# orishu/kraken

Hardware: AMD Instinct MI355X
Metric: metainfo+digest GB/s (device-resident & end-to-end) at 1/2/4/8 MI355X (higher is better)
Workload: dtype u8

## Files before the change

### kraken_amd/csrc/sha256_multi.hip

```cpp
#include <stdlib.h>

#include <atomic>
#include <mutex>

#include "../../include/kraken_hip_internal.h"
#include "kernels.hpp"
#include "knobs.hpp"
#include "device_util.hpp"

namespace krk {

#define KRK_K256                                                                                 \
    0x428a2f98u, 0x71374491u, 0xb5c0fbcfu, 0xe9b5dba5u, 0x3956c25bu, 0x59f111f1u, 0x923f82a4u,     \
        0xab1c5ed5u, 0xd807aa98u, 0x12835b01u, 0x243185beu, 0x550c7dc3u, 0x72be5d74u, 0x80deb1feu, \
        0x9bdc06a7u, 0xc19bf174u, 0xe49b69c1u, 0xefbe4786u, 0x0fc19dc6u, 0x240ca1ccu, 0x2de92c6fu, \
        0x4a7484aau, 0x5cb0a9dcu, 0x76f988dau, 0x983e5152u, 0xa831c66du, 0xb00327c8u, 0xbf597fc7u, \
        0xc6e00bf3u, 0xd5a79147u, 0x06ca6351u, 0x14292967u, 0x27b70a85u, 0x2e1b2138u, 0x4d2c6dfcu, \
        0x53380d13u, 0x650a7354u, 0x766a0abbu, 0x81c2c92eu, 0x92722c85u, 0xa2bfe8a1u, 0xa81a664bu, \
        0xc24b8b70u, 0xc76c51a3u, 0xd192e819u, 0xd6990624u, 0xf40e3585u, 0x106aa070u, 0x19a4c116u, \
        0x1e376c08u, 0x2748774cu, 0x34b0bcb5u, 0x391c0cb3u, 0x4ed8aa4au, 0x5b9cca4fu, 0x682e6ff3u, \
        0x748f82eeu, 0x78a5636fu, 0x84c87814u, 0x8cc70208u, 0x90befffau, 0xa4506cebu, 0xbef9a3f7u, \
        0xc67178f2u

__device__ __forceinline__ uint32_t rotr(uint32_t x, uint32_t n) {
    return __builtin_amdgcn_alignbit(x, x, n);
}
__device__ __forceinline__ uint32_t bswap(uint32_t x) { return __builtin_bswap32(x); }

#ifdef KRK_DIAG
__device__ __forceinline__ void compress(uint32_t h[8], uint32_t w[16]) {
    constexpr uint32_t K[64] = {KRK_K256};
    uint32_t a = h[0], b = h[1], c = h[2], d = h[3], e = h[4], f = h[5], g = h[6], hh = h[7];
#pragma unroll
    for (int i = 0; i < 64; ++i) {
        uint32_t wi;
        if (i < 16) {
            wi = w[i];
        } else {
            const uint32_t w15 = w[(i - 15) & 15], w2 = w[(i - 2) & 15];
            const uint32_t s0 = xor3(rotr(w15, 7), rotr(w15, 18), w15 >> 3);
            const uint32_t s1 = xor3(rotr(w2, 17), rotr(w2, 19), w2 >> 10);
            wi = w[i & 15] + s0 + w[(i - 7) & 15] + s1;
            w[i & 15] = wi;
        }
        const uint32_t S1 = xor3(rotr(e, 6), rotr(e, 11), rotr(e, 25));
        const uint32_t ch = (e & f) ^ (~e & g);
        const uint32_t t1 = hh + S1 + ch + K[i] + wi;
        const uint32_t S0 = xor3(rotr(a, 2), rotr(a, 13), rotr(a, 22));
        const uint32_t mj = __builtin_amdgcn_bitop3_b32(a, b, c, 0xE8);
        const uint32_t t2 = S0 + mj;
        hh = g; g = f; f = e; e = d + t1; d = c; c = b; b = a; a = t1 + t2;
    }
    h[0] += a; h[1] += b; h[2] += c; h[3] += d; h[4] += e; h[5] += f; h[6] += g; h[7] += hh;
}

__device__ __forceinline__ void load_block(uint64_t p, bool al16, uint32_t w[16], uint64_t lo = 0,
                                           uint64_t hi = ~0ull) {
    if (al16) {
        gptr<u32x4> q = as_global<u32x4>(p);
#pragma unroll
        for (int k = 0; k < 4; ++k) {
            const u32x4 v = KRK_GUARD(p + 16 * k, 16, lo, hi, 2) ? q[k] : u32x4{0, 0, 0, 0};
            w[4 * k + 0] = bswap(v.x); w[4 * k + 1] = bswap(v.y);
            w[4 * k + 2] = bswap(v.z); w[4 * k + 3] = bswap(v.w);
        }
    } else {
        load_bytes64(p, 64, w, lo, hi);
#pragma unroll
        for (int k = 0; k < 16; ++k) w[k] = bswap(w[k]);
    }
}

__global__ void __launch_bounds__(64)
sha256_multi_kernel(const ShaJob* __restrict__ jobs, uint32_t n_jobs, uint8_t* __restrict__ out_digest,
                    uint32_t* __restrict__ out_state) {
    const uint32_t j = blockIdx.x * 64 + threadIdx.x;
    if (j >= n_jobs) return;
    const ShaJob job = jobs[j];
    const uint64_t p = job.ptr;
    const bool al16 = (job.ptr & 15) == 0;
    const uint64_t lo = p & ~uint64_t(3), hi = (p + job.len + 3) & ~uint64_t(3);
    uint32_t h[8];
    if (job.flags & kShaFromState) {
#pragma unroll
        for (int k = 0; k < 8; ++k) h[k] = out_state[8 * (uint64_t)job.out + k];
    } else {
// ... 181 lines not shown
#define KRK_SHA_ROUND(A, B, C, D, E, F, G, HK, KWN, NE, NA, NH)                  \
    "v_alignbit_b32 %[r6], %[" #E "], %[" #E "], 6\n\t"                        \
    "v_alignbit_b32 %[r11], %[" #E "], %[" #E "], 11\n\t"                      \
    "v_alignbit_b32 %[r25], %[" #E "], %[" #E "], 25\n\t"                      \
    "v_bitop3_b32 %[ch], %[" #E "], %[" #F "], %[" #G "] bitop3:0xca\n\t"     \
    "v_bitop3_b32 %[r6], %[r6], %[r11], %[r25] bitop3:0x96\n\t"                \
    "v_alignbit_b32 %[q2], %[" #A "], %[" #A "], 2\n\t"                        \
    "v_add3_u32 %[t1], %[" #HK "], %[r6], %[ch]\n\t"                           \
    "v_alignbit_b32 %[q13], %[" #A "], %[" #A "], 13\n\t"                      \
    "v_add_u32_e32 %[" #NE "], %[" #D "], %[t1]\n\t"                           \
    "v_alignbit_b32 %[q22], %[" #A "], %[" #A "], 22\n\t"                      \
    "v_bitop3_b32 %[mj], %[" #A "], %[" #B "], %[" #C "] bitop3:0xe8\n\t"     \
    "v_bitop3_b32 %[q2], %[q2], %[q13], %[q22] bitop3:0x96\n\t"                \
    "v_add_u32_e32 %[" #NH "], %[" #G "], %[" #KWN "]\n\t"                     \
    "v_add3_u32 %[" #NA "], %[t1], %[q2], %[mj]\n\t"

__device__ __forceinline__ void sha_quad(uint32_t& a, uint32_t& b, uint32_t& c, uint32_t& d, uint32_t& e,
                                         uint32_t& f, uint32_t& g, uint32_t& hk, uint32_t k1, uint32_t k2,
                                         uint32_t k3, uint32_t k4, uint32_t& h_last) {
    uint32_t r6, r11, r25, ch, q2, t1, q13, q22, mj;
    uint32_t e1, e2, e3, e4, a1, a2, a3, a4, h1, h2, h3, h4;
    asm volatile(KRK_SHA_ROUND(a, b, c, d, e, f, g, hk, k1, e1, a1, h1)
                 KRK_SHA_ROUND(a1, a, b, c, e1, e, f, h1, k2, e2, a2, h2)
                 KRK_SHA_ROUND(a2, a1, a, b, e2, e1, e, h2, k3, e3, a3, h3)
                 KRK_SHA_ROUND(a3, a2, a1, a, e3, e2, e1, h3, k4, e4, a4, h4)
                 : [r6] "=&v"(r6), [r11] "=&v"(r11), [r25] "=&v"(r25), [ch] "=&v"(ch), [q2] "=&v"(q2),
                   [t1] "=&v"(t1), [q13] "=&v"(q13), [q22] "=&v"(q22), [mj] "=&v"(mj), [e1] "=&v"(e1),
                   [e2] "=&v"(e2), [e3] "=&v"(e3), [e4] "=&v"(e4), [a1] "=&v"(a1), [a2] "=&v"(a2),
                   [a3] "=&v"(a3), [a4] "=&v"(a4), [h1] "=&v"(h1), [h2] "=&v"(h2), [h3] "=&v"(h3),
                   [h4] "=&v"(h4)
                 : [a] "v"(a), [b] "v"(b), [c] "v"(c), [d] "v"(d), [e] "v"(e), [f] "v"(f), [g] "v"(g),
                   [hk] "v"(hk), [k1] "v"(k1), [k2] "v"(k2), [k3] "v"(k3), [k4] "v"(k4));
    h_last = e1;
    a = a4; b = a3; c = a2; d = a1;
    e = e4; f = e3; g = e2;
    hk = h4;
}
#undef KRK_SHA_ROUND

__device__ __forceinline__ void rounds(uint32_t h[8], const uint32_t* lds, int slot, uint32_t lane,
                                       const u32x4& k0, const u32x4& k1) {
    uint32_t a = h[0], b = h[1], c = h[2], d = h[3], e = h[4], f = h[5], g = h[6];
    uint32_t hk = h[7] + k0[0], hl = 0;
    u32x4 kw = k0, nkw = k1, nnkw = k1;
#pragma unroll
    for (int q = 0; q < 16; ++q) {
        if (q + 2 < 16) nnkw = *reinterpret_cast<const u32x4*>(lds + kw_index(slot, q + 2, lane));
        sha_quad(a, b, c, d, e, f, g, hk, kw[1], kw[2], kw[3], q + 1 < 16 ? nkw[0] : 0u, hl);
        kw = nkw;
        nkw = nnkw;
    }
    h[0] += a; h[1] += b; h[2] += c; h[3] += d; h[4] += e; h[5] += f; h[6] += g; h[7] += hl;
}

__device__ __forceinline__ u32x4 kw_quad(const uint32_t* lds, int slot, int q, uint32_t lane) {
    return *reinterpret_cast<const u32x4*>(lds + kw_index(slot, q, lane));
}

__device__ __forceinline__ bool two_lane_is_e(uint32_t lane) { return (lane >> 3) & 1; }
__device__ __forceinline__ uint32_t two_lane_stream(uint32_t lane) {
    return (lane >> 4) * 8 + (two_lane_is_e(lane) ? 7 - (lane & 7) : (lane & 7));
}

#define KRK_SHA2_ROUND(X0, X1, X2, NX, WN)                                              \
    "v_add_u32_dpp %[p], %[" #X1 "], %[z] row_mirror row_mask:0xf bank_mask:0xf\n\t"    \
    "v_alignbit_b32 %[t1], %[" #X0 "], %[" #X0 "], %[r1]\n\t"                          \
    "v_alignbit_b32 %[t2], %[" #X0 "], %[" #X0 "], %[r2]\n\t"                          \
    "v_alignbit_b32 %[t3], %[" #X0 "], %[" #X0 "], %[r3]\n\t"                          \
    "v_bitop3_b32 %[k], %[" #X0 "], %[" #X1 "], %[ma] bitop3:0x2d\n\t"                 \
    "v_bitop3_b32 %[t1], %[t1], %[t2], %[t3] bitop3:0x96\n\t"                          \
    "v_bitop3_b32 %[k], %[k], %[" #X2 "], %[" #X1 "] bitop3:0xca\n\t"                  \
    "v_xad_u32 %[z], %[" #X2 "], %[ma], %[" #WN "]\n\t"                                \
    "v_add3_u32 %[" #NX "], %[t1], %[k], %[p]\n\t"

struct TwoLaneConst {
    uint32_t r1, r2, r3, ma, one_a;
};

#define KRK_SHA2_OPERANDS                                                                             \
    : [t1] "=&v"(t1), [t2] "=&v"(t2), [t3] "=&v"(t3), [k] "=&v"(kk), [p] "=&v"(p), [z] "+v"(z),       \
      [R0] "+v"(R0), [R1] "+v"(R1), [R2] "+v"(R2), [R3] "+v"(R3)
#define KRK_SHA2_CONSTS [r1] "v"(c.r1), [r2] "v"(c.r2), [r3] "v"(c.r3), [ma] "v"(c.ma)

#define KRK_SHA8_ROUND(X0, X1, X2, NX, WN)                                                   \
    "v_alignbit_b32 %[t1], %[" #X0 "], %[" #X0 "], %[r1]\n\t"                               \
    "v_bitop3_b32 %[k], %[" #X0 "], %[" #X1 "], %[ma] bitop3:0x2d\n\t"                      \
    "v_bitop3_b32 %[k], %[k], %[" #X2 "], %[" #X1 "] bitop3:0xca\n\t"                       \
    "v_xor_b32_dpp %[t2], %[t1], %[t1] quad_perm:[1,2,0,3] row_mask:0xf bank_mask:0xf\n\t"  \
    "v_xor_b32_dpp %[t2], %[t1], %[t2] quad_perm:[2,0,1,3] row_mask:0xf bank_mask:0xf\n\t"  \
    "v_add_u32_dpp %[p], %[" #X1 "], %[z] row_ror:8 row_mask:0xf bank_mask:0xf\n\t"          \
    "v_xad_u32 %[z], %[" #X2 "], %[ma], %[" #WN "]\n\t"                                     \
    "v_add3_u32 %[" #NX "], %[t2], %[k], %[p]\n\t"
#define KRK_SHA8_OPERANDS                                                                    \
    : [t1] "=&v"(t1), [t2] "=&v"(t2), [k] "=&v"(kk), [p] "=&v"(p), [z] "+v"(z), [R0] "+v"(R0), \
      [R1] "+v"(R1), [R2] "+v"(R2), [R3] "+v"(R3)
#define KRK_SHA8_CONSTS [r1] "v"(c.r1), [ma] "v"(c.ma)

__device__ __forceinline__ void sha2_quad(uint32_t& R0, uint32_t& R1, uint32_t& R2, uint32_t& R3, uint32_t& z,
                                          const TwoLaneConst& c, uint32_t w1, uint32_t w2, uint32_t w3,
                                          uint32_t w4) {
    uint32_t t1, t2, t3, kk, p;
    asm volatile(KRK_SHA2_ROUND(R0, R3, R2, R1, w1)
                 KRK_SHA2_ROUND(R1, R0, R3, R2, w2)
                 KRK_SHA2_ROUND(R2, R1, R0, R3, w3)
                 KRK_SHA2_ROUND(R3, R2, R1, R0, w4)
                 KRK_SHA2_OPERANDS
                 : KRK_SHA2_CONSTS, [w1] "v"(w1), [w2] "v"(w2), [w3] "v"(w3), [w4] "v"(w4));
    (void)t3;
}

#define KRK_SHA_AHEAD 3
constexpr int kAhead = KRK_SHA_AHEAD;
#define KRK_SHA8_UNROLL 4
static_assert(kAhead >= 2 && kAhead <= 8, "read-ahead distance");

__device__ __forceinline__ void sha8_quad2(uint32_t& R0, uint32_t& R1, uint32_t& R2, uint32_t& R3, uint32_t& z,
                                           const TwoLaneConst& c, uint32_t w1, uint32_t w2, uint32_t w3,
                                           uint32_t w4) {
    uint32_t t1, t2, kk, p;
    asm volatile(KRK_SHA8_ROUND(R2, R1, R0, R3, w1) KRK_SHA8_ROUND(R3, R2, R1, R0, w2)
                 KRK_SHA8_ROUND(R0, R3, R2, R1, w3) KRK_SHA8_ROUND(R1, R0, R3, R2, w4)
                 KRK_SHA8_OPERANDS
                 : KRK_SHA8_CONSTS, [w1] "v"(w1), [w2] "v"(w2), [w3] "v"(w3), [w4] "v"(w4));
}

constexpr int kAhead8 = 4;
__device__ __forceinline__ void sha8_dodec2(uint32_t& R0, uint32_t& R1, uint32_t& R2, uint32_t& R3, uint32_t& z,
                                            const TwoLaneConst& c, const u32x4& a, const u32x4& b, const u32x4& d,
                                            const u32x4& e) {
    uint32_t t1, t2, kk, p;
    asm volatile(KRK_SHA8_ROUND(R2, R1, R0, R3, w1) KRK_SHA8_ROUND(R3, R2, R1, R0, w2)
                 KRK_SHA8_ROUND(R0, R3, R2, R1, w3) KRK_SHA8_ROUND(R1, R0, R3, R2, w4)
                 KRK_SHA8_ROUND(R2, R1, R0, R3, w5) KRK_SHA8_ROUND(R3, R2, R1, R0, w6)
                 KRK_SHA8_ROUND(R0, R3, R2, R1, w7) KRK_SHA8_ROUND(R1, R0, R3, R2, w8)
                 KRK_SHA8_ROUND(R2, R1, R0, R3, w9) KRK_SHA8_ROUND(R3, R2, R1, R0, w10)
                 KRK_SHA8_ROUND(R0, R3, R2, R1, w11) KRK_SHA8_ROUND(R1, R0, R3, R2, w12)
                 KRK_SHA8_OPERANDS
                 : KRK_SHA8_CONSTS, [w1] "v"(a[3]), [w2] "v"(b[0]), [w3] "v"(b[1]), [w4] "v"(b[2]),
                   [w5] "v"(b[3]), [w6] "v"(d[0]), [w7] "v"(d[1]), [w8] "v"(d[2]), [w9] "v"(d[3]),
                   [w10] "v"(e[0]), [w11] "v"(e[1]), [w12] "v"(e[2]));
}

__device__ __forceinline__ void block8p(uint32_t& R0, uint32_t& R1, uint32_t& R2, uint32_t& R3, uint32_t& z,
                                        uint32_t hE[4], uint32_t hA[4], uint32_t mineE, uint32_t mineA,
                                        uint32_t i, const uint32_t* lds, uint32_t cbase, uint32_t nbase,
                                        const TwoLaneConst& c, u32x4 k[kAhead8]) {
    constexpr int kRS = kAhead8 + 1;
    u32x4 wq[kRS];
#pragma unroll
    for (int j = 0; j < kAhead8; ++j) wq[j] = k[j];
    constexpr int RS = kAhead8 + 3;
    u32x4 wr[RS];
#pragma unroll
    for (int j = 0; j < kAhead8; ++j) wr[j] = wq[j];
    auto rd = [&](int q) {
        if (q < 16) wr[q % RS] = *reinterpret_cast<const u32x4*>(lds + cbase + 256 * q);
        else k[q - 16] = *reinterpret_cast<const u32x4*>(lds + nbase + 256 * (q - 16));
    };
#pragma unroll
    for (int j = 0; j < 15; j += 3) {
        rd(j + kAhead8);
        rd(j + kAhead8 + 1);
        rd(j + kAhead8 + 2);
        sha8_dodec2(R0, R1, R2, R3, z, c, wr[j % RS], wr[(j + 1) % RS], wr[(j + 2) % RS], wr[(j + 3) % RS]);
    }
    wq[15 % kRS] = wr[15 % RS];
    k[kAhead8 - 1] = *reinterpret_cast<const u32x4*>(lds + nbase + 256 * (kAhead8 - 1));
    {
        uint32_t t1, t2, kk, p;
        asm volatile(KRK_SHA8_ROUND(R2, R1, R0, R3, w3)
                     KRK_SHA8_ROUND(R3, R2, R1, R0, w4)
                     KRK_SHA8_OPERANDS
                     : KRK_SHA8_CONSTS, [w3] "v"(wq[15 % kRS][3]), [w4] "v"(k[0][0]));
    }
    {
        uint32_t t1, t2, kk, p, cc, dd, c2;
        asm volatile("v_sub_u32_e32 %[cc], %[a0], %[e0]\n\t"
                     "v_sub_u32_e32 %[dd], %[a1], %[e1]\n\t"
                     "v_add_u32_e32 %[R0], %[e0], %[R0]\n\t"
                     "v_add_u32_e32 %[R3], %[e1], %[R3]\n\t"
                     "v_mov_b32_dpp %[c2], %[cc] row_ror:8 row_mask:0xf bank_mask:0xf\n\t"
                     "v_add_u32_dpp %[z], %[dd], %[z] row_ror:8 row_mask:0xf bank_mask:0xf\n\t"
                     "v_add_u32_e32 %[R2], %[e2], %[R2]\n\t"
                     "v_add_u32_e32 %[R1], %[e3], %[R1]\n\t"
                     "v_add_u32_e32 %[z], %[e3], %[z]\n\t"
                     "v_cmp_lt_u32_e32 vcc, %[i], %[mineE]\n\t"
                     "v_cndmask_b32_e32 %[e0], %[e0], %[R0], vcc\n\t"
                     "v_cndmask_b32_e32 %[e1], %[e1], %[R3], vcc\n\t"
                     "v_cndmask_b32_e32 %[e2], %[e2], %[R2], vcc\n\t"
                     "v_cndmask_b32_e32 %[e3], %[e3], %[R1], vcc\n\t"
                     KRK_SHA8_ROUND(R0, R3, R2, R1, w1)
                     "v_add_u32_e32 %[z], %[c2], %[z]\n\t"
                     KRK_SHA8_ROUND(R1, R0, R3, R2, w2)
                     "v_sub_u32_e32 %[z], %[z], %[a1]\n\t"
                     "v_add_u32_e32 %[R0], %[a0], %[R0]\n\t"
                     "v_add_u32_e32 %[R3], %[a1], %[R3]\n\t"
                     "v_add_u32_e32 %[R2], %[a2], %[R2]\n\t"
                     "v_add_u32_e32 %[R1], %[a3], %[R1]\n\t"
                     "v_cmp_lt_u32_e32 vcc, %[i], %[mineA]\n\t"
                     "v_cndmask_b32_e32 %[a0], %[a0], %[R0], vcc\n\t"
                     "v_cndmask_b32_e32 %[a1], %[a1], %[R3], vcc\n\t"
                     "v_cndmask_b32_e32 %[a2], %[a2], %[R2], vcc\n\t"
                     "v_cndmask_b32_e32 %[a3], %[a3], %[R1], vcc\n\t"
                     : [t1] "=&v"(t1), [t2] "=&v"(t2), [k] "=&v"(kk), [p] "=&v"(p), [cc] "=&v"(cc), [dd] "=&v"(dd),
                       [c2] "=&v"(c2), [z] "+v"(z),
                       [R0] "+v"(R0), [R1] "+v"(R1), [R2] "+v"(R2), [R3] "+v"(R3), [e0] "+v"(hE[0]),
                       [e1] "+v"(hE[1]), [e2] "+v"(hE[2]), [e3] "+v"(hE[3]), [a0] "+v"(hA[0]), [a1] "+v"(hA[1]),
                       [a2] "+v"(hA[2]), [a3] "+v"(hA[3])
                     : KRK_SHA8_CONSTS, [w1] "v"(k[0][1]), [w2] "v"(k[0][2]), [i] "s"(i), [mineE] "v"(mineE),
                       [mineA] "v"(mineA)
                     : "vcc");
    }
}

__device__ __forceinline__ void prologue8p(uint32_t& R0, uint32_t& R1, uint32_t& R2, uint32_t& R3, uint32_t& z,
                                           const uint32_t h[4], bool is_e, const TwoLaneConst& c,
                                           const u32x4& k0) {
    {
        uint32_t t1, t2, kk, p;
        asm volatile("v_xad_u32 %[z], %[R1], %[ma], %[w0]\n\t"
                     KRK_SHA8_ROUND(R0, R3, R2, R1, w1)
                     KRK_SHA8_OPERANDS
                     : KRK_SHA8_CONSTS, [w0] "v"(k0[0]), [w1] "v"(k0[1]));
    }
    R1 = is_e ? R1 : h[3];
    {
        uint32_t t1, t2, kk, p;
        asm volatile(KRK_SHA8_ROUND(R1, R0, R3, R2, w2)
                     KRK_SHA8_OPERANDS
                     : KRK_SHA8_CONSTS, [w2] "v"(k0[2]));
    }
    R2 = is_e ? R2 : h[2];
}
__device__ __forceinline__ void sha2_quad2(uint32_t& R0, uint32_t& R1, uint32_t& R2, uint32_t& R3, uint32_t& z,
                                           const TwoLaneConst& c, uint32_t w1, uint32_t w2, uint32_t w3,
                                           uint32_t w4) {
    uint32_t t1, t2, t3, kk, p;
    asm volatile(KRK_SHA2_ROUND(R2, R1, R0, R3, w1) KRK_SHA2_ROUND(R3, R2, R1, R0, w2)
                 KRK_SHA2_ROUND(R0, R3, R2, R1, w3) KRK_SHA2_ROUND(R1, R0, R3, R2, w4)
                 KRK_SHA2_OPERANDS
                 : KRK_SHA2_CONSTS, [w1] "v"(w1), [w2] "v"(w2), [w3] "v"(w3), [w4] "v"(w4));
}

constexpr int kAhead2 = 4;
__device__ __forceinline__ void sha2_dodec2(uint32_t& R0, uint32_t& R1, uint32_t& R2, uint32_t& R3, uint32_t& z,
                                            const TwoLaneConst& c, const u32x4& a, const u32x4& b, const u32x4& d,
                                            const u32x4& e) {
    uint32_t t1, t2, t3, kk, p;
    asm volatile(KRK_SHA2_ROUND(R2, R1, R0, R3, w1) KRK_SHA2_ROUND(R3, R2, R1, R0, w2)
                 KRK_SHA2_ROUND(R0, R3, R2, R1, w3) KRK_SHA2_ROUND(R1, R0, R3, R2, w4)
                 KRK_SHA2_ROUND(R2, R1, R0, R3, w5) KRK_SHA2_ROUND(R3, R2, R1, R0, w6)
                 KRK_SHA2_ROUND(R0, R3, R2, R1, w7) KRK_SHA2_ROUND(R1, R0, R3, R2, w8)
                 KRK_SHA2_ROUND(R2, R1, R0, R3, w9) KRK_SHA2_ROUND(R3, R2, R1, R0, w10)
                 KRK_SHA2_ROUND(R0, R3, R2, R1, w11) KRK_SHA2_ROUND(R1, R0, R3, R2, w12)
                 KRK_SHA2_OPERANDS
                 : KRK_SHA2_CONSTS, [w1] "v"(a[3]), [w2] "v"(b[0]), [w3] "v"(b[1]), [w4] "v"(b[2]),
                   [w5] "v"(b[3]), [w6] "v"(d[0]), [w7] "v"(d[1]), [w8] "v"(d[2]), [w9] "v"(d[3]),
                   [w10] "v"(e[0]), [w11] "v"(e[1]), [w12] "v"(e[2]));
    (void)t3;
}


__device__ __forceinline__ void block2p(uint32_t& R0, uint32_t& R1, uint32_t& R2, uint32_t& R3, uint32_t& z,
                                        uint32_t hE[4], uint32_t hA[4], uint32_t mineE, uint32_t mineA,
                                        uint32_t i, const uint32_t* lds, uint32_t cbase, uint32_t nbase,
                                        const TwoLaneConst& c, u32x4 k[kAhead2]) {
    constexpr int kRS = kAhead2 + 1;
    u32x4 wq[kRS];
#pragma unroll
    for (int j = 0; j < kAhead2; ++j) wq[j] = k[j];
    constexpr int RS = kAhead2 + 3;
    u32x4 wr[RS];
#pragma unroll
    for (int j = 0; j < kAhead2; ++j) wr[j] = wq[j];
    auto rd = [&](int q) {
        if (q < 16) wr[q % RS] = *reinterpret_cast<const u32x4*>(lds + cbase + 256 * q);
        else k[q - 16] = *reinterpret_cast<const u32x4*>(lds + nbase + 256 * (q - 16));
    };
#pragma unroll
    for (int j = 0; j < 15; j += 3) {
        rd(j + kAhead2);
        rd(j + kAhead2 + 1);
        rd(j + kAhead2 + 2);
        sha2_dodec2(R0, R1, R2, R3, z, c, wr[j % RS], wr[(j + 1) % RS], wr[(j + 2) % RS], wr[(j + 3) % RS]);
    }
    wq[15 % kRS] = wr[15 % RS];
    k[kAhead2 - 1] = *reinterpret_cast<const u32x4*>(lds + nbase + 256 * (kAhead2 - 1));
    {
        uint32_t t1, t2, t3, kk, p;
        asm volatile(KRK_SHA2_ROUND(R2, R1, R0, R3, w3)
                     KRK_SHA2_ROUND(R3, R2, R1, R0, w4)
                     KRK_SHA2_OPERANDS
                     : KRK_SHA2_CONSTS, [w3] "v"(wq[15 % kRS][3]), [w4] "v"(k[0][0]));
    }
    {
        uint32_t t1, t2, t3, kk, p, cc, dd, c2, w1c;
// ... 236 lines not shown
                    reinterpret_cast<uint4*>(o)[1] = make_uint4(bswap(h[4]), bswap(h[5]), bswap(h[6]), bswap(h[7]));
                } else {
                    for (int k = 0; k < 32; ++k) o[k] = (uint8_t)(h[k >> 2] >> (24 - 8 * (k & 3)));
                }
            } else {
                uint32_t* o = out_state + 8 * (uint64_t)job.out;
#pragma unroll
                for (int k = 0; k < 8; ++k) o[k] = h[k];
            }
        }
    }
}

template <int kTiming, int kGroups>
__global__ void __launch_bounds__(128 * kGroups)
sha256_w8_kernel(const ShaJob* __restrict__ jobs, uint32_t n_jobs, uint8_t* __restrict__ out_digest,
                 uint32_t* __restrict__ out_state) {
    extern __shared__ __attribute__((aligned(16))) uint32_t ring_all[];
    constexpr int kStep8 = 8, kRing8 = 3, kNs = kStep8 * kRing8;
    constexpr uint32_t kPer = 8;
    constexpr uint32_t kRingWords = uint32_t(kRing8 + 1) * kSlotWords + kOnesPad8;
    const uint32_t lane = threadIdx.x & 63;
    const uint32_t wave = threadIdx.x >> 6;
    const bool producer = wave < (uint32_t)kGroups;
    const uint32_t grp = wave % kGroups;
    uint32_t* ring = ring_all + grp * kRingWords;
    const uint32_t sbase = blockIdx.x * kPer * kGroups;
    const uint32_t quad = (lane >> 2) & 3;
    const uint32_t me = producer ? (lane & 7) : (lane >> 4) * 2 + (quad & 1);
    const uint32_t j = sbase + grp * kPer + me;
    const bool live = j < n_jobs;
    ShaJob job{};
    if (live) job = jobs[j];
    const uint32_t mine = live ? job_blocks(job) : 0u;
    uint32_t nb = 0;
#pragma unroll
    for (int g = 0; g < kGroups; ++g) {
        const uint32_t jj = sbase + g * kPer + me;
        if (jj < n_jobs) nb = max(nb, g == (int)grp ? mine : job_blocks(jobs[jj]));
    }
#pragma unroll
    for (int off = 32; off > 0; off >>= 1) nb = max(nb, (uint32_t)__shfl_xor((int)nb, off, 64));
    nb = __builtin_amdgcn_readfirstlane(nb);

    if (producer && kTiming == 1) return;
    if (producer) {
#pragma unroll
        for (int q = 0; q < 16; ++q) *reinterpret_cast<u32x4*>(ring + kw_index(kRing8, q, lane)) = u32x4{1u, 1u, 1u, 1u};
        *reinterpret_cast<u32x4*>(ring + (kRing8 + 1) * kSlotWords + lane * 4) = u32x4{1u, 1u, 1u, 1u};
        u32x4 R0[kRaw], R1[kRaw], R2[kRaw];
        const uint64_t safe = reinterpret_cast<uint64_t>(jobs);
        const uint32_t par = lane >> 3;
        uint32_t passed = 0;
        fetch(job, par, R0, safe);
        fetch(job, par + kStep8, R1, safe);
        for (uint32_t b = 0; b < nb; b += 3 * kStep8) {
            produce_step<kNs, kStep8>(job, b, b + par, nb, lane, ring, R0, R2, safe, passed);
            produce_step<kNs, kStep8>(job, b + kStep8, b + kStep8 + par, nb, lane, ring, R1, R0, safe, passed);
            produce_step<kNs, kStep8>(job, b + 2 * kStep8, b + 2 * kStep8 + par, nb, lane, ring, R2, R1, safe, passed);
        }
        while (passed < (nb + kStep8 - 1) / kStep8) {
            __syncthreads();
            ++passed;
        }
        return;
    }
    const bool is_e = quad < 2;
    const uint32_t pos = lane & 3;
    const uint32_t half = is_e ? 4u : 0u;
    const uint32_t r1 = is_e ? (pos == 1 ? 11u : pos == 2 ? 25u : 6u) : (pos == 1 ? 13u : pos == 2 ? 22u : 2u);
    const TwoLaneConst c{r1, 0u, 0u, is_e ? 0u : ~0u, is_e ? 0u : 1u};
    uint32_t h[4];
    if (live && (job.flags & kShaFromState)) {
#pragma unroll
        for (int k = 0; k < 4; ++k) h[k] = out_state[8 * (uint64_t)job.out + half + (is_e ? k : k ^ 2)];
    } else {
#pragma unroll
        for (int k = 0; k < 4; ++k) h[k] = is_e ? job.h[4 + k] : job.h[k ^ 2];
    }
    __builtin_amdgcn_s_setprio(3);
    const uint32_t lbase = is_e ? me * 4u : uint32_t(kRing8) * kSlotWords + 32u;
    const uint32_t binc = 32u, sinc = is_e ? uint32_t(kSlotWords) : 0u;
    uint32_t voff = 0, vslot = 0, slot = 0;
    u32x4 kq[kAhead8] = {};
    uint32_t hE[4], hA[4];
#pragma unroll
    for (int k = 0; k < 4; ++k) {
        hE[k] = is_e ? h[k] : 0u;
        hA[k] = is_e ? 0u : h[k];
    }
    const uint32_t mineE = is_e ? mine : 0u, mineA = is_e ? 0u : mine;
    uint32_t R0 = h[0], R3 = h[1], R2 = h[2], R1 = h[3], z = 0;
    auto block = [&](uint32_t i, uint32_t cur, uint32_t nxt) {
        block8p(R0, R1, R2, R3, z, hE, hA, mineE, mineA, i, ring, cur, nxt, c, kq);
    };
    constexpr uint32_t kU = KRK_SHA8_UNROLL;
    static_assert(kU == 1 || kU == 2 || kU == 4 || kU == 8, "blocks per iteration divide a step");
    if (nb) {
        if (kTiming == 0) __builtin_amdgcn_s_barrier();
        asm volatile("" ::: "memory");
#pragma unroll
        for (int q = 0; q < kAhead8; ++q) kq[q] = *reinterpret_cast<const u32x4*>(ring + lbase + 256 * q);
        prologue8p(R0, R1, R2, R3, z, h, is_e, c, kq[0]);
    }
    for (uint32_t i = 0; i < nb; i += kU) {
        const uint32_t jj = i & (kStep8 - 1);
        if (jj == 0 && i) {
            if (kTiming == 0) __builtin_amdgcn_s_barrier();
            asm volatile("" ::: "memory");
        }
        const bool last = jj == kStep8 - kU;
        const uint32_t nvslot = slot == kRing8 - 1 ? 0u : vslot + sinc;
        uint32_t o = voff;
#pragma unroll
        for (uint32_t u = 0; u < kU; ++u) {
            const uint32_t on = (u == kU - 1 && last) ? nvslot : o + binc;
            if (u == 0 || i + u < nb) block(i + u, lbase + o, lbase + on);
            o = on;
        }
        voff = o;
        if (last) {
            slot = slot == kRing8 - 1 ? 0u : slot + 1;
            vslot = nvslot;
        }
    }
#pragma unroll
    for (int k = 0; k < 4; ++k) h[k] = is_e ? hE[k] : hA[k];
    if (live && pos == 0) {
        uint32_t hs[4];
#pragma unroll
        for (int k = 0; k < 4; ++k) hs[k] = is_e ? h[k] : h[k ^ 2];
        if (job.flags & kShaFinal) {
            uint8_t* o = out_digest + 32 * (uint64_t)job.out + 4 * half;
            if ((reinterpret_cast<uintptr_t>(o) & 15) == 0) {
                reinterpret_cast<uint4*>(o)[0] = make_uint4(bswap(hs[0]), bswap(hs[1]), bswap(hs[2]), bswap(hs[3]));
            } else {
                for (int k = 0; k < 16; ++k) o[k] = (uint8_t)(hs[k >> 2] >> (24 - 8 * (k & 3)));
            }
        } else {
            uint32_t* o = out_state + 8 * (uint64_t)job.out + half;
#pragma unroll
            for (int k = 0; k < 4; ++k) o[k] = hs[k];
        }
    }
}

static std::atomic<int> g_sha_plan{-1};

static int sha_plan() {
    int p = g_sha_plan.load(std::memory_order_relaxed);
    if (p >= 0) return p;
    const char* e = KRK_AB_ENV("KRK_SHA_PLAN");
    int want = e ? atoi(e) : KRK_SHA_PLAN_AUTO;
    if (!sha_plan_valid(want)) want = KRK_SHA_PLAN_AUTO;
    int expect = -1;
    g_sha_plan.compare_exchange_strong(expect, want);
    return g_sha_plan.load(std::memory_order_relaxed);
}

bool sha_plan_valid(int p) {
    if (p >= KRK_SHA_PLAN_AUTO && p <= KRK_SHA_PLAN_8LANE_2PAIR) return true;
#ifdef KRK_DIAG
    return p >= 100 && p <= 108;
#else
    return false;
#endif
}

void set_sha_plan(int p) { g_sha_plan.store(p, std::memory_order_relaxed); }

static uint32_t device_cus() {
    static uint32_t n = [] {
        int dev = 0, cus = 256;
        if (hipGetDevice(&dev) == hipSuccess) {
            hipDeviceProp_t p;
            if (hipGetDeviceProperties(&p, dev) == hipSuccess && p.multiProcessorCount > 0) cus = p.multiProcessorCount;
        }
        return (uint32_t)cus;
    }();
    return n;
}
static uint32_t two_lane_max_streams() { return device_cus() * 64u; }

static int auto_plan(uint32_t n_jobs) {
    if (n_jobs <= device_cus() * 16u) return KRK_SHA_PLAN_8LANE;
    if (n_jobs <= device_cus() * 32u) return KRK_SHA_PLAN_2LANE;
    return n_jobs <= two_lane_max_streams() ? KRK_SHA_PLAN_2LANE_2PAIR : KRK_SHA_PLAN_1LANE_2PAIR;
}

static int resolve_plan(uint32_t n_jobs) {
    const int p = sha_plan();
    return p == KRK_SHA_PLAN_AUTO ? auto_plan(n_jobs) : p;
}

static bool plan_two_lanes(int p) {
    return p == KRK_SHA_PLAN_2LANE || p == KRK_SHA_PLAN_2LANE_2PAIR || p == 103 || p == 104 || p == 106 ||
           p == 107;
}

static bool plan_eight_lanes(int p) { return p == KRK_SHA_PLAN_8LANE || p == KRK_SHA_PLAN_8LANE_2PAIR || p == 108; }

int sha_plan_for(uint32_t n_jobs) { return resolve_plan(n_jobs); }

int sha_lanes_for(uint32_t n_jobs) {
    const int p = resolve_plan(n_jobs);
    return plan_eight_lanes(p) ? 8 : plan_two_lanes(p) ? 2 : 1;
}

// ... 93 lines not shown
```

Baseline: 58.99.

## Hand-schedule SHA-256 block LDS reads into pinned VGPRs with burst prefetch

Replaces the compiler-scheduled per-block message loads and 12-round asm chunks with one inline-asm block per SHA block. It issues ds_read_b128 bursts into fixed VGPRs v64–v127 and waits on them with explicit lgkmcnt. Nine quads of the next block are held across block boundaries, and LDS offsets become immediate template constants, so the compiler's read scheduling and address arithmetic go away. In exchange it pins 64 VGPRs by hand and relies on manual s_waitcnt placement. That raises register pressure and the risk of reading before the data has landed.

```diff
diff --git a/kraken_amd/csrc/sha256_multi.hip b/kraken_amd/csrc/sha256_multi.hip
--- a/kraken_amd/csrc/sha256_multi.hip
+++ b/kraken_amd/csrc/sha256_multi.hip
@@ -2,6 +2,7 @@
 
 #include <atomic>
 #include <mutex>
+#include <type_traits>
 
 #include "../../include/kraken_hip_internal.h"
 #include "kernels.hpp"
@@ -349,14 +350,15 @@
       [R0] "+v"(R0), [R1] "+v"(R1), [R2] "+v"(R2), [R3] "+v"(R3)
 #define KRK_SHA2_CONSTS [r1] "v"(c.r1), [r2] "v"(c.r2), [r3] "v"(c.r3), [ma] "v"(c.ma)
 
-#define KRK_SHA8_ROUND(X0, X1, X2, NX, WN)                                                   \
+#define KRK_SHA8_ROUND(X0, X1, X2, NX, WN) KRK_SHA8_ROUND_(X0, X1, X2, NX, "%[" #WN "]")
+#define KRK_SHA8_ROUND_(X0, X1, X2, NX, W)                                                   \
     "v_alignbit_b32 %[t1], %[" #X0 "], %[" #X0 "], %[r1]\n\t"                               \
     "v_bitop3_b32 %[k], %[" #X0 "], %[" #X1 "], %[ma] bitop3:0x2d\n\t"                      \
     "v_bitop3_b32 %[k], %[k], %[" #X2 "], %[" #X1 "] bitop3:0xca\n\t"                       \
     "v_xor_b32_dpp %[t2], %[t1], %[t1] quad_perm:[1,2,0,3] row_mask:0xf bank_mask:0xf\n\t"  \
     "v_xor_b32_dpp %[t2], %[t1], %[t2] quad_perm:[2,0,1,3] row_mask:0xf bank_mask:0xf\n\t"  \
     "v_add_u32_dpp %[p], %[" #X1 "], %[z] row_ror:8 row_mask:0xf bank_mask:0xf\n\t"          \
-    "v_xad_u32 %[z], %[" #X2 "], %[ma], %[" #WN "]\n\t"                                     \
+    "v_xad_u32 %[z], %[" #X2 "], %[ma], " W "\n\t"                                          \
     "v_add3_u32 %[" #NX "], %[t2], %[k], %[p]\n\t"
 #define KRK_SHA8_OPERANDS                                                                    \
     : [t1] "=&v"(t1), [t2] "=&v"(t2), [k] "=&v"(kk), [p] "=&v"(p), [z] "+v"(z), [R0] "+v"(R0), \
@@ -381,104 +383,91 @@
 #define KRK_SHA8_UNROLL 4
 static_assert(kAhead >= 2 && kAhead <= 8, "read-ahead distance");
 
-__device__ __forceinline__ void sha8_quad2(uint32_t& R0, uint32_t& R1, uint32_t& R2, uint32_t& R3, uint32_t& z,
-                                           const TwoLaneConst& c, uint32_t w1, uint32_t w2, uint32_t w3,
-                                           uint32_t w4) {
-    uint32_t t1, t2, kk, p;
-    asm volatile(KRK_SHA8_ROUND(R2, R1, R0, R3, w1) KRK_SHA8_ROUND(R3, R2, R1, R0, w2)
-                 KRK_SHA8_ROUND(R0, R3, R2, R1, w3) KRK_SHA8_ROUND(R1, R0, R3, R2, w4)
-                 KRK_SHA8_OPERANDS
-                 : KRK_SHA8_CONSTS, [w1] "v"(w1), [w2] "v"(w2), [w3] "v"(w3), [w4] "v"(w4));
-}
-
-constexpr int kAhead8 = 4;
-__device__ __forceinline__ void sha8_dodec2(uint32_t& R0, uint32_t& R1, uint32_t& R2, uint32_t& R3, uint32_t& z,
-                                            const TwoLaneConst& c, const u32x4& a, const u32x4& b, const u32x4& d,
-                                            const u32x4& e) {
-    uint32_t t1, t2, kk, p;
-    asm volatile(KRK_SHA8_ROUND(R2, R1, R0, R3, w1) KRK_SHA8_ROUND(R3, R2, R1, R0, w2)
-                 KRK_SHA8_ROUND(R0, R3, R2, R1, w3) KRK_SHA8_ROUND(R1, R0, R3, R2, w4)
-                 KRK_SHA8_ROUND(R2, R1, R0, R3, w5) KRK_SHA8_ROUND(R3, R2, R1, R0, w6)
-                 KRK_SHA8_ROUND(R0, R3, R2, R1, w7) KRK_SHA8_ROUND(R1, R0, R3, R2, w8)
-                 KRK_SHA8_ROUND(R2, R1, R0, R3, w9) KRK_SHA8_ROUND(R3, R2, R1, R0, w10)
-                 KRK_SHA8_ROUND(R0, R3, R2, R1, w11) KRK_SHA8_ROUND(R1, R0, R3, R2, w12)
-                 KRK_SHA8_OPERANDS
-                 : KRK_SHA8_CONSTS, [w1] "v"(a[3]), [w2] "v"(b[0]), [w3] "v"(b[1]), [w4] "v"(b[2]),
-                   [w5] "v"(b[3]), [w6] "v"(d[0]), [w7] "v"(d[1]), [w8] "v"(d[2]), [w9] "v"(d[3]),
-                   [w10] "v"(e[0]), [w11] "v"(e[1]), [w12] "v"(e[2]));
-}
-
+constexpr int kHeld8 = 9;
+#define KRK_SHA8_RD(Q0, Q1, BASE, OFF, Q) \
+    "ds_read_b128 v[" #Q0 ":" #Q1 "], %[" #BASE "] offset:%[" #OFF "]+" #Q "*1024\n\t"
+#define KRK_SHA8_QT(W1, W2, W3, W4, B)                                                \
+    KRK_SHA8_ROUND_(R2, R1, R0, R3, #W1) B KRK_SHA8_ROUND_(R3, R2, R1, R0, #W2)      \
+    KRK_SHA8_ROUND_(R0, R3, R2, R1, #W3) KRK_SHA8_ROUND_(R1, R0, R3, R2, #W4)
+#define KRK_SHA8_BURST_A                                                                          \
+    "s_waitcnt lgkmcnt(0)\n\t"                                                                    \
+    KRK_SHA8_RD(100, 103, cb, co, 9) KRK_SHA8_RD(104, 107, cb, co, 10) KRK_SHA8_RD(108, 111, cb, co, 11) \
+    KRK_SHA8_RD(112, 115, cb, co, 12) KRK_SHA8_RD(116, 119, cb, co, 13) KRK_SHA8_RD(120, 123, cb, co, 14) \
+    KRK_SHA8_RD(124, 127, cb, co, 15) KRK_SHA8_RD(64, 67, nb, no, 0)
+#define KRK_SHA8_BURST_B                                                                          \
+    "s_waitcnt lgkmcnt(0)\n\t"                                                                    \
+    KRK_SHA8_RD(68, 71, nb, no, 1) KRK_SHA8_RD(72, 75, nb, no, 2) KRK_SHA8_RD(76, 79, nb, no, 3)   \
+    KRK_SHA8_RD(80, 83, nb, no, 4) KRK_SHA8_RD(84, 87, nb, no, 5) KRK_SHA8_RD(88, 91, nb, no, 6)   \
+    KRK_SHA8_RD(92, 95, nb, no, 7) KRK_SHA8_RD(96, 99, nb, no, 8)
+
+template <uint32_t kCurOff, uint32_t kNxtOff>
 __device__ __forceinline__ void block8p(uint32_t& R0, uint32_t& R1, uint32_t& R2, uint32_t& R3, uint32_t& z,
                                         uint32_t hE[4], uint32_t hA[4], uint32_t mineE, uint32_t mineA,
-                                        uint32_t i, const uint32_t* lds, uint32_t cbase, uint32_t nbase,
-                                        const TwoLaneConst& c, u32x4 k[kAhead8]) {
-    constexpr int kRS = kAhead8 + 1;
-    u32x4 wq[kRS];
-#pragma unroll
-    for (int j = 0; j < kAhead8; ++j) wq[j] = k[j];
-    constexpr int RS = kAhead8 + 3;
-    u32x4 wr[RS];
-#pragma unroll
-    for (int j = 0; j < kAhead8; ++j) wr[j] = wq[j];
-    auto rd = [&](int q) {
-        if (q < 16) wr[q % RS] = *reinterpret_cast<const u32x4*>(lds + cbase + 256 * q);
-        else k[q - 16] = *reinterpret_cast<const u32x4*>(lds + nbase + 256 * (q - 16));
-    };
-#pragma unroll
-    for (int j = 0; j < 15; j += 3) {
-        rd(j + kAhead8);
-        rd(j + kAhead8 + 1);
-        rd(j + kAhead8 + 2);
-        sha8_dodec2(R0, R1, R2, R3, z, c, wr[j % RS], wr[(j + 1) % RS], wr[(j + 2) % RS], wr[(j + 3) % RS]);
-    }
-    wq[15 % kRS] = wr[15 % RS];
-    k[kAhead8 - 1] = *reinterpret_cast<const u32x4*>(lds + nbase + 256 * (kAhead8 - 1));
-    {
-        uint32_t t1, t2, kk, p;
-        asm volatile(KRK_SHA8_ROUND(R2, R1, R0, R3, w3)
-                     KRK_SHA8_ROUND(R3, R2, R1, R0, w4)
-                     KRK_SHA8_OPERANDS
-                     : KRK_SHA8_CONSTS, [w3] "v"(wq[15 % kRS][3]), [w4] "v"(k[0][0]));
-    }
-    {
-        uint32_t t1, t2, kk, p, cc, dd, c2;
-        asm volatile("v_sub_u32_e32 %[cc], %[a0], %[e0]\n\t"
-                     "v_sub_u32_e32 %[dd], %[a1], %[e1]\n\t"
-                     "v_add_u32_e32 %[R0], %[e0], %[R0]\n\t"
-                     "v_add_u32_e32 %[R3], %[e1], %[R3]\n\t"
-                     "v_mov_b32_dpp %[c2], %[cc] row_ror:8 row_mask:0xf bank_mask:0xf\n\t"
-                     "v_add_u32_dpp %[z], %[dd], %[z] row_ror:8 row_mask:0xf bank_mask:0xf\n\t"
-                     "v_add_u32_e32 %[R2], %[e2], %[R2]\n\t"
-                     "v_add_u32_e32 %[R1], %[e3], %[R1]\n\t"
-                     "v_add_u32_e32 %[z], %[e3], %[z]\n\t"
-                     "v_cmp_lt_u32_e32 vcc, %[i], %[mineE]\n\t"
-                     "v_cndmask_b32_e32 %[e0], %[e0], %[R0], vcc\n\t"
-                     "v_cndmask_b32_e32 %[e1], %[e1], %[R3], vcc\n\t"
-                     "v_cndmask_b32_e32 %[e2], %[e2], %[R2], vcc\n\t"
-                     "v_cndmask_b32_e32 %[e3], %[e3], %[R1], vcc\n\t"
-                     KRK_SHA8_ROUND(R0, R3, R2, R1, w1)
-                     "v_add_u32_e32 %[z], %[c2], %[z]\n\t"
-                     KRK_SHA8_ROUND(R1, R0, R3, R2, w2)
-                     "v_sub_u32_e32 %[z], %[z], %[a1]\n\t"
-                     "v_add_u32_e32 %[R0], %[a0], %[R0]\n\t"
-                     "v_add_u32_e32 %[R3], %[a1], %[R3]\n\t"
-                     "v_add_u32_e32 %[R2], %[a2], %[R2]\n\t"
-                     "v_add_u32_e32 %[R1], %[a3], %[R1]\n\t"
-                     "v_cmp_lt_u32_e32 vcc, %[i], %[mineA]\n\t"
-                     "v_cndmask_b32_e32 %[a0], %[a0], %[R0], vcc\n\t"
-                     "v_cndmask_b32_e32 %[a1], %[a1], %[R3], vcc\n\t"
-                     "v_cndmask_b32_e32 %[a2], %[a2], %[R2], vcc\n\t"
-                     "v_cndmask_b32_e32 %[a3], %[a3], %[R1], vcc\n\t"
-                     : [t1] "=&v"(t1), [t2] "=&v"(t2), [k] "=&v"(kk), [p] "=&v"(p), [cc] "=&v"(cc), [dd] "=&v"(dd),
-                       [c2] "=&v"(c2), [z] "+v"(z),
-                       [R0] "+v"(R0), [R1] "+v"(R1), [R2] "+v"(R2), [R3] "+v"(R3), [e0] "+v"(hE[0]),
-                       [e1] "+v"(hE[1]), [e2] "+v"(hE[2]), [e3] "+v"(hE[3]), [a0] "+v"(hA[0]), [a1] "+v"(hA[1]),
-                       [a2] "+v"(hA[2]), [a3] "+v"(hA[3])
-                     : KRK_SHA8_CONSTS, [w1] "v"(k[0][1]), [w2] "v"(k[0][2]), [i] "s"(i), [mineE] "v"(mineE),
-                       [mineA] "v"(mineA)
-                     : "vcc");
-    }
-}
+                                        uint32_t i, uint32_t cur, uint32_t nxt, const TwoLaneConst& c,
+                                        u32x4 k[kHeld8]) {
+    uint32_t t1, t2, kk, p, cc, dd, c2;
+    asm volatile(KRK_SHA8_QT(v67, v68, v69, v70, KRK_SHA8_BURST_A)
+                 KRK_SHA8_QT(v71, v72, v73, v74, "")
+                 KRK_SHA8_QT(v75, v76, v77, v78, "")
+                 KRK_SHA8_QT(v79, v80, v81, v82, "")
+                 KRK_SHA8_QT(v83, v84, v85, v86, "")
+                 KRK_SHA8_QT(v87, v88, v89, v90, "")
+                 KRK_SHA8_QT(v91, v92, v93, v94, "")
+                 KRK_SHA8_QT(v95, v96, v97, v98, "")
+                 KRK_SHA8_QT(v99, v100, v101, v102, KRK_SHA8_BURST_B)
+                 KRK_SHA8_QT(v103, v104, v105, v106, "")
+                 KRK_SHA8_QT(v107, v108, v109, v110, "")
+                 KRK_SHA8_QT(v111, v112, v113, v114, "")
+                 KRK_SHA8_QT(v115, v116, v117, v118, "")
+                 KRK_SHA8_QT(v119, v120, v121, v122, "")
+                 KRK_SHA8_QT(v123, v124, v125, v126, "")
+                 KRK_SHA8_ROUND_(R2, R1, R0, R3, "v127")
+                 KRK_SHA8_ROUND_(R3, R2, R1, R0, "v64")
+                 "v_sub_u32_e32 %[cc], %[a0], %[e0]\n\t"
+                 "v_sub_u32_e32 %[dd], %[a1], %[e1]\n\t"
+                 "v_add_u32_e32 %[R0], %[e0], %[R0]\n\t"
+                 "v_add_u32_e32 %[R3], %[e1], %[R3]\n\t"
+                 "v_mov_b32_dpp %[c2], %[cc] row_ror:8 row_mask:0xf bank_mask:0xf\n\t"
+                 "v_add_u32_dpp %[z], %[dd], %[z] row_ror:8 row_mask:0xf bank_mask:0xf\n\t"
+                 "v_add_u32_e32 %[R2], %[e2], %[R2]\n\t"
+                 "v_add_u32_e32 %[R1], %[e3], %[R1]\n\t"
+                 "v_add_u32_e32 %[z], %[e3], %[z]\n\t"
+                 "v_cmp_lt_u32_e32 vcc, %[i], %[mineE]\n\t"
+                 "v_cndmask_b32_e32 %[e0], %[e0], %[R0], vcc\n\t"
+                 "v_cndmask_b32_e32 %[e1], %[e1], %[R3], vcc\n\t"
+                 "v_cndmask_b32_e32 %[e2], %[e2], %[R2], vcc\n\t"
+                 "v_cndmask_b32_e32 %[e3], %[e3], %[R1], vcc\n\t"
+                 KRK_SHA8_ROUND_(R0, R3, R2, R1, "v65")
+                 "v_add_u32_e32 %[z], %[c2], %[z]\n\t"
+                 KRK_SHA8_ROUND_(R1, R0, R3, R2, "v66")
+                 "v_sub_u32_e32 %[z], %[z], %[a1]\n\t"
+                 "v_add_u32_e32 %[R0], %[a0], %[R0]\n\t"
+                 "v_add_u32_e32 %[R3], %[a1], %[R3]\n\t"
+                 "v_add_u32_e32 %[R2], %[a2], %[R2]\n\t"
+                 "v_add_u32_e32 %[R1], %[a3], %[R1]\n\t"
+                 "v_cmp_lt_u32_e32 vcc, %[i], %[mineA]\n\t"
+                 "v_cndmask_b32_e32 %[a0], %[a0], %[R0], vcc\n\t"
+                 "v_cndmask_b32_e32 %[a1], %[a1], %[R3], vcc\n\t"
+                 "v_cndmask_b32_e32 %[a2], %[a2], %[R2], vcc\n\t"
+                 "v_cndmask_b32_e32 %[a3], %[a3], %[R1], vcc\n\t"
+                 : [t1] "=&v"(t1), [t2] "=&v"(t2), [k] "=&v"(kk), [p] "=&v"(p), [cc] "=&v"(cc), [dd] "=&v"(dd),
+                   [c2] "=&v"(c2), [z] "+v"(z),
+                   [R0] "+v"(R0), [R1] "+v"(R1), [R2] "+v"(R2), [R3] "+v"(R3), [e0] "+v"(hE[0]),
+                   [e1] "+v"(hE[1]), [e2] "+v"(hE[2]), [e3] "+v"(hE[3]), [a0] "+v"(hA[0]), [a1] "+v"(hA[1]),
+                   [a2] "+v"(hA[2]), [a3] "+v"(hA[3]),
+                   "+{v[64:67]}"(k[0]), "+{v[68:71]}"(k[1]), "+{v[72:75]}"(k[2]), "+{v[76:79]}"(k[3]),
+                   "+{v[80:83]}"(k[4]), "+{v[84:87]}"(k[5]), "+{v[88:91]}"(k[6]), "+{v[92:95]}"(k[7]),
+                   "+{v[96:99]}"(k[8])
+                 : KRK_SHA8_CONSTS, [i] "s"(i), [mineE] "v"(mineE), [mineA] "v"(mineA), [cb] "v"(cur),
+                   [nb] "v"(nxt), [co] "n"(kCurOff), [no] "n"(kNxtOff)
+                 : "vcc", "memory", "v100", "v101", "v102", "v103", "v104", "v105", "v106", "v107", "v108",
+                   "v109", "v110", "v111", "v112", "v113", "v114", "v115", "v116", "v117", "v118", "v119", "v120",
+                   "v121", "v122", "v123", "v124", "v125", "v126", "v127");
+}
+#undef KRK_SHA8_QT
+#undef KRK_SHA8_BURST_A
+#undef KRK_SHA8_BURST_B
+#undef KRK_SHA8_RD
 
 __device__ __forceinline__ void prologue8p(uint32_t& R0, uint32_t& R1, uint32_t& R2, uint32_t& R3, uint32_t& z,
                                            const uint32_t h[4], bool is_e, const TwoLaneConst& c,
@@ -881,7 +870,8 @@
     const uint32_t lbase = is_e ? me * 4u : uint32_t(kRing8) * kSlotWords + 32u;
     const uint32_t binc = 32u, sinc = is_e ? uint32_t(kSlotWords) : 0u;
     uint32_t voff = 0, vslot = 0, slot = 0;
-    u32x4 kq[kAhead8] = {};
+    const uint32_t lbyte = (uint32_t)(uintptr_t)(__attribute__((address_space(3))) uint32_t*)ring + 4u * lbase;
+    u32x4 kq[kHeld8] = {};
     uint32_t hE[4], hA[4];
 #pragma unroll
     for (int k = 0; k < 4; ++k) {
@@ -890,16 +880,13 @@
     }
     const uint32_t mineE = is_e ? mine : 0u, mineA = is_e ? 0u : mine;
     uint32_t R0 = h[0], R3 = h[1], R2 = h[2], R1 = h[3], z = 0;
-    auto block = [&](uint32_t i, uint32_t cur, uint32_t nxt) {
-        block8p(R0, R1, R2, R3, z, hE, hA, mineE, mineA, i, ring, cur, nxt, c, kq);
-    };
     constexpr uint32_t kU = KRK_SHA8_UNROLL;
     static_assert(kU == 1 || kU == 2 || kU == 4 || kU == 8, "blocks per iteration divide a step");
     if (nb) {
         if (kTiming == 0) __builtin_amdgcn_s_barrier();
         asm volatile("" ::: "memory");
 #pragma unroll
-        for (int q = 0; q < kAhead8; ++q) kq[q] = *reinterpret_cast<const u32x4*>(ring + lbase + 256 * q);
+        for (int q = 0; q < kHeld8; ++q) kq[q] = *reinterpret_cast<const u32x4*>(ring + lbase + 256 * q);
         prologue8p(R0, R1, R2, R3, z, h, is_e, c, kq[0]);
     }
     for (uint32_t i = 0; i < nb; i += kU) {
@@ -910,19 +897,40 @@
         }
         const bool last = jj == kStep8 - kU;
         const uint32_t nvslot = slot == kRing8 - 1 ? 0u : vslot + sinc;
-        uint32_t o = voff;
-#pragma unroll
-        for (uint32_t u = 0; u < kU; ++u) {
-            const uint32_t on = (u == kU - 1 && last) ? nvslot : o + binc;
-            if (u == 0 || i + u < nb) block(i + u, lbase + o, lbase + on);
-            o = on;
-        }
-        voff = o;
+        const uint32_t cur = lbyte + 4u * voff;
+        voff = last ? nvslot : voff + kU * binc;
+        const uint32_t nxt = lbyte + 4u * voff;
+        auto block = [&](auto u) {
+            constexpr uint32_t kB = 4u * binc * decltype(u)::value;
+            if constexpr (decltype(u)::value == kU - 1) {
+                block8p<kB, 0>(R0, R1, R2, R3, z, hE, hA, mineE, mineA, i + u, cur, nxt, c, kq);
+            } else {
+                block8p<kB, kB + 4u * binc>(R0, R1, R2, R3, z, hE, hA, mineE, mineA, i + u, cur, cur, c, kq);
+            }
+        };
+        block(std::integral_constant<uint32_t, 0>{});
+        if constexpr (kU > 1) if (i + 1 < nb) block(std::integral_constant<uint32_t, 1 % kU>{});
+        if constexpr (kU > 2) {
+            if (i + 2 < nb) block(std::integral_constant<uint32_t, 2 % kU>{});
+            if (i + 3 < nb) block(std::integral_constant<uint32_t, 3 % kU>{});
+        }
+        if constexpr (kU > 4) {
+            if (i + 4 < nb) block(std::integral_constant<uint32_t, 4 % kU>{});
+            if (i + 5 < nb) block(std::integral_constant<uint32_t, 5 % kU>{});
+            if (i + 6 < nb) block(std::integral_constant<uint32_t, 6 % kU>{});
+            if (i + 7 < nb) block(std::integral_constant<uint32_t, 7 % kU>{});
+        }
         if (last) {
             slot = slot == kRing8 - 1 ? 0u : slot + 1;
             vslot = nvslot;
         }
     }
+    asm volatile("s_waitcnt lgkmcnt(0)"
+                 : "+{v[64:67]}"(kq[0]), "+{v[68:71]}"(kq[1]), "+{v[72:75]}"(kq[2]), "+{v[76:79]}"(kq[3]),
+                   "+{v[80:83]}"(kq[4]), "+{v[84:87]}"(kq[5]), "+{v[88:91]}"(kq[6]), "+{v[92:95]}"(kq[7]),
+                   "+{v[96:99]}"(kq[8])
+                 :
+                 : "memory");
 #pragma unroll
     for (int k = 0; k < 4; ++k) h[k] = is_e ? hE[k] : hA[k];
     if (live && pos == 0) {
```

New measurement: 59.87 (median of 6 runs). +1.5%, better.
